# Yusheng-Xu/VGS-SVGS-Segmentation

Measured on AMD Instinct MI355X. Metric: segmented points/sec (end-to-end VGS), higher is better.
Workload: dtype f32

## Files before the change

vgs-svgs-segmentation_amd/csrc/capi.hip:

```cpp
#include <algorithm>
#include <cstdio>
#include <cstdlib>
#include <cstring>
#include <fstream>
#include <string>
#include <vector>

#include <dlfcn.h>

#include "vgs_context.hpp"

static thread_local std::string g_create_err;

static const char* const VGS_STAGE_NAMES[VGS_T_COUNT] = {"vgs:voxelize", "vgs:features", "vgs:adjacency", "vgs:localcut", "vgs:merge", "vgs:labels",
                                                         "vgs:total", "vgs:localcut_kernel", "vgs:supervoxels", "vgs:localcut_bulk", "", ""};
struct RoctxApi {
  int (*push)(const char*) = nullptr;
  int (*pop)() = nullptr;
  RoctxApi() {
    for (const char* name : {"librocprofiler-sdk-roctx.so.1", "librocprofiler-sdk-roctx.so", "libroctx64.so.4", "libroctx64.so"}) {
      void* h = dlopen(name, RTLD_LAZY | RTLD_LOCAL);
      if (!h) continue;
      push = (int (*)(const char*))dlsym(h, "roctxRangePushA");
      pop = (int (*)())dlsym(h, "roctxRangePop");
// ... 92 lines not shown
  }
  auto num = [&](size_t k) -> double { return k < v.size() ? std::atof(v[k].c_str()) : 0.0; };
  auto inum = [&](size_t k) -> int { return k < v.size() ? std::atoi(v[k].c_str()) : 0; };
  if (v.size() < 51) return VGS_E_IO;
  const int method = inum(24);
  if (method == 3) {
    if (v.size() < 61) return VGS_E_IO;
    vgs_params_default_svgs(p);
    p->voxel_size = (float)num(28); p->seed_size = (float)num(30); p->graph_size = (float)num(32);
    p->sig_p = (float)num(34); p->sig_n = (float)num(36); p->sig_o = (float)num(38); p->sig_e = (float)num(40);
    p->sig_c = (float)num(42); p->sig_w = (float)num(44);
    p->color_impt = (float)num(46); p->spatial_impt = (float)num(48); p->normal_impt = (float)num(50);
    p->cut_thred = (float)num(52);
    p->points_min = (int)num(54); p->voxels_min = inum(58); p->adjacency_min = inum(60);
  } else {
    vgs_params_default_vgs(p);
    p->voxel_size = (float)num(28); p->graph_size = (float)num(30);
    p->sig_p = (float)num(32); p->sig_n = (float)num(34); p->sig_o = (float)num(36); p->sig_e = (float)num(38);
    p->sig_c = (float)num(40); p->sig_w = (float)num(42); p->cut_thred = (float)num(44);
    p->points_min = inum(46); p->adjacency_min = inum(48); p->voxels_min = inum(50);
    p->method = 2;
  }
  if (in_name && name_cap > 0) { std::strncpy(in_name, v[15].c_str(), name_cap - 1); in_name[name_cap - 1] = 0; }
  if (out_name && name_cap > 0) { std::strncpy(out_name, v[21].c_str(), name_cap - 1); out_name[name_cap - 1] = 0; }
  return VGS_OK;
}

vgs_status vgs_create(const vgs_params* p, vgs_ctx** out) {
  if (!p || !out) return VGS_E_ARG;
  *out = nullptr;
  if (!(p->voxel_size > 0.f) || !(p->graph_size > 0.f) || !(p->sig_w != 0.f) || (p->method != 2 && p->method != 3)) {
    g_create_err = "vgs_create: voxel_size, graph_size must be > 0, sig_w != 0, method 2 or 3";
    return VGS_E_ARG;
  }
  if (p->vccs_mode != 0 && p->vccs_mode != 1) { g_create_err = "vgs_create: vccs_mode must be 0 (synchronous variant) or 1 (PCL's order)"; return VGS_E_ARG; }
  int ndev = 0;
  hipError_t e = hipGetDeviceCount(&ndev);
  if (e != hipSuccess || ndev <= 0) {
    g_create_err = std::string("vgs_create: no HIP device (") + hipGetErrorString(e) + "); this engine has no CPU path";
    return VGS_E_HIP;
  }
  if (p->device < 0 || p->device >= ndev) { g_create_err = "vgs_create: bad device ordinal"; return VGS_E_ARG; }
  vgs_ctx* c = new (std::nothrow) vgs_ctx();
  if (!c) return VGS_E_NOMEM;
  c->P = *p;
  c->device = p->device;
  int prio_lo = 0, prio_hi = 0;
  if (hipSetDevice(c->device) != hipSuccess || hipStreamCreateWithFlags(&c->stream, hipStreamNonBlocking) != hipSuccess ||
      hipDeviceGetStreamPriorityRange(&prio_lo, &prio_hi) != hipSuccess ||
      hipStreamCreateWithPriority(&c->stream2, hipStreamNonBlocking, prio_hi) != hipSuccess ||
      hipStreamCreateWithPriority(&c->stream3, hipStreamNonBlocking, prio_hi) != hipSuccess ||
      hipStreamCreateWithPriority(&c->stream4, hipStreamNonBlocking, prio_hi) != hipSuccess) {
    g_create_err = "vgs_create: hipSetDevice/hipStreamCreate failed";
    vgs_destroy(c);
    return VGS_E_HIP;
  }
  if (hipHostMalloc(&c->pin, 4096, hipHostMallocDefault) != hipSuccess) c->pin = nullptr;
  bool ok = hipStreamCreateWithFlags(&c->s_h2d, hipStreamNonBlocking) == hipSuccess &&
            hipStreamCreateWithFlags(&c->s_d2h, hipStreamNonBlocking) == hipSuccess &&
            hipEventCreateWithFlags(&c->ev_h2d, hipEventDisableTiming) == hipSuccess &&
            hipEventCreateWithFlags(&c->ev_d2h, hipEventDisableTiming) == hipSuccess &&
            hipEventCreateWithFlags(&c->ev_rb, hipEventDisableTiming) == hipSuccess &&
            hipEventCreateWithFlags(&c->ev_ho, hipEventDisableTiming) == hipSuccess &&
            hipEventCreateWithFlags(&c->ev_ho2, hipEventDisableTiming) == hipSuccess;
  for (int i = 0; ok && i < 16; ++i) ok = hipEventCreate(&c->ev[i]) == hipSuccess;
  for (int i = 0; ok && i < VGS_T_COUNT; ++i) ok = hipEventCreate(&c->tev[i][0]) == hipSuccess && hipEventCreate(&c->tev[i][1]) == hipSuccess;
  if (!ok) { g_create_err = "vgs_create: hipStreamCreate/hipEventCreate failed"; vgs_destroy(c); return VGS_E_HIP; }
  vgs_read_env_knobs(c);
  *out = c;
  return VGS_OK;
}

void vgs_destroy(vgs_ctx* c) {
  if (!c) return;
  (void)hipSetDevice(c->device);
  if (c->stream) (void)hipStreamSynchronize(c->stream);
  if (c->stream2) (void)hipStreamSynchronize(c->stream2);
  if (c->stream3) (void)hipStreamSynchronize(c->stream3);
  if (c->stream4) (void)hipStreamSynchronize(c->stream4);
  if (c->s_h2d) (void)hipStreamSynchronize(c->s_h2d);
  if (c->s_d2h) (void)hipStreamSynchronize(c->s_d2h);
  c->xyz_buf[0].release(); c->xyz_buf[1].release(); c->pt_label_alt.release(); c->grow_state.release();
  c->code_a.release(); c->code_b.release(); c->perm_a.release(); c->perm_b.release(); c->sort_tmp.release();
  c->head_flag.release(); c->pt_vox.release(); c->vox_code.release(); c->vox_start.release();
  c->xs.release(); c->ys.release(); c->zs.release();
  c->node.release(); c->used_ids.release(); c->used_rank.release();
  c->hkey.release(); c->hval.release(); c->offsets.release(); c->adj_masks.release(); c->adj_gtab.release(); c->adj_nvals.release(); c->adj_nrank.release(); c->adj_key.release(); c->adj_off.release(); c->adj_cnt.release(); c->adj_mused.release();
  c->nl_cnt.release(); c->nl_tot.release(); c->nl_ent.release(); c->lc_ctab.release(); c->pl_state.release(); c->pl_ent.release(); c->pl_work.release();
  c->sd_key.release(); c->sd_ids.release(); c->sd_vp.release(); c->sd_seg.release(); c->sd_tmp.release(); c->sd_part.release();
  c->sd_npts.release(); c->sd_nnodes.release(); c->sd_bbox.release(); c->sd_eig8.release(); c->sd_cen.release(); c->sd_cov.release(); c->sd_eval.release(); c->sd_evec.release();
  c->sd_apos.release(); c->sd_mom.release();
  c->sg_lab.release(); c->sg_nrec.release(); c->sg_ridx.release(); c->sg_ework.release(); c->sg_meta.release(); c->sg_roff.release(); c->sg_rkey.release(); c->sg_rec.release(); c->sg_part.release(); c->sg_tmp.release();
  c->sg_ab.release(); c->sg_nodes.release(); c->sg_npairs.release(); c->sg_nfin.release(); c->sg_wsum.release(); c->sg_wmin.release(); c->sg_wmax.release();
  c->cl_off.release(); c->cl_idx.release(); c->conn.release(); c->evals.release(); c->lc_pending.release(); c->lc_defer.release(); c->lc_defer_flag.release(); c->csize.release(); c->attach.release(); c->cc_flags.release(); c->parent.release(); c->csz.release();
  c->vc_cen.release(); c->vc_nrm.release(); c->vc_dist.release(); c->vc_state.release(); c->vc_tile_start.release(); c->vc_cell.release(); c->vc_plive.release(); c->vc_tile_of.release(); c->vc_tchg.release(); c->vc_nbr_tiles.release(); c->vc_halo.release(); c->vc_tile_meta.release(); c->vc_pool.release(); c->vc_ring.release(); c->vc_dbg.release(); c->vc_label.release();
  c->vc_seedkey.release(); c->vc_sums.release(); c->vc_count.release(); c->vc_accu.release(); c->vc_alive.release();
  c->sv_label.release(); c->sv_key_a.release(); c->sv_key_b.release(); c->cell_code_a.release(); c->cell_code_b.release();
  c->cell_id_a.release(); c->cell_id_b.release(); c->cell_start.release();
  c->owned.release(); c->straddle.release(); c->mixsrc.release(); c->bnd_code.release(); c->bnd_root.release(); c->root_label.release();
  c->bnd_code2.release(); c->bnd_root2.release(); c->bnd_cnt.release(); c->broot.release();
  c->kept_rank.release(); c->vox_label.release(); c->pt_label.release(); c->counters.release(); c->work_ids.release();
  if (c->pin) (void)hipHostFree(c->pin);
  for (int i = 0; i < 16; ++i) if (c->ev[i]) (void)hipEventDestroy(c->ev[i]);
  for (int i = 0; i < VGS_T_COUNT; ++i) for (int k = 0; k < 2; ++k) if (c->tev[i][k]) (void)hipEventDestroy(c->tev[i][k]);
  if (c->stream) (void)hipStreamDestroy(c->stream);
  if (c->stream2) (void)hipStreamDestroy(c->stream2);
  if (c->stream3) (void)hipStreamDestroy(c->stream3);
  if (c->stream4) (void)hipStreamDestroy(c->stream4);
  if (c->s_h2d) (void)hipStreamDestroy(c->s_h2d);
  if (c->s_d2h) (void)hipStreamDestroy(c->s_d2h);
  if (c->ev_h2d) (void)hipEventDestroy(c->ev_h2d);
  if (c->ev_rb) (void)hipEventDestroy(c->ev_rb);
  if (c->ev_ho) (void)hipEventDestroy(c->ev_ho);
  if (c->ev_ho2) (void)hipEventDestroy(c->ev_ho2);
  if (c->ev_d2h) (void)hipEventDestroy(c->ev_d2h);
  delete c;
}

vgs_status vgs_set_params(vgs_ctx* c, const vgs_params* p) {
  if (!c || !p) return VGS_E_ARG;
  if (!(p->voxel_size > 0.f) || !(p->graph_size > 0.f) || !(p->sig_w != 0.f)) { c->err = "vgs_set_params: voxel_size, graph_size > 0, sig_w != 0"; return VGS_E_ARG; }
  if (p->method != c->P.method || p->device != c->P.device) { c->err = "vgs_set_params: method and device are fixed at vgs_create"; return VGS_E_ARG; }
  if (p->vccs_mode != 0 && p->vccs_mode != 1) { c->err = "vgs_set_params: vccs_mode must be 0 (synchronous variant) or 1 (PCL's order)"; return VGS_E_ARG; }
  int keep = ST_SEGMENTED;
  const vgs_params& o = c->P;
  if (p->cut_thred != o.cut_thred || p->sig_p != o.sig_p || p->sig_n != o.sig_n || p->sig_o != o.sig_o || p->sig_e != o.sig_e ||
      p->sig_c != o.sig_c || p->sig_w != o.sig_w || p->adjacency_min != o.adjacency_min || p->voxels_min != o.voxels_min ||
      p->q7_count_as_index != o.q7_count_as_index)
    keep = ST_ADJACENCY;
  if (p->graph_size != o.graph_size) keep = ST_FEATURES;
  if (p->points_min != o.points_min) keep = ST_VOXELS;
  if (p->voxel_size != o.voxel_size || p->seed_size != o.seed_size || p->color_impt != o.color_impt ||
      p->spatial_impt != o.spatial_impt || p->normal_impt != o.normal_impt || p->vccs_mode != o.vccs_mode)
    keep = ST_POINTS;
  if (c->stage > keep) c->stage = keep;
  if (keep < ST_SEGMENTED) { c->sd_valid = false; c->sg_valid = false; c->sg_halo_valid = false; c->sg_own_K = -1; }
  if (keep == ST_POINTS && c->P.method == 3 && !c->sv_labels_external) { c->sv_have_labels = false; c->sv_max_label = 0; c->sv_label_n = -1; }
  c->P = *p;
  return VGS_OK;
}

const char* vgs_last_error_string(const vgs_ctx* c) { return c ? c->err.c_str() : g_create_err.c_str(); }

static vgs_status set_points_common(vgs_ctx* c, int64_t n, int32_t stride_bytes) {
  if (n < 0 || (stride_bytes != 12 && stride_bytes != 16)) { c->err = "set_points: n >= 0 and stride_bytes 12 or 16 required"; return VGS_E_ARG; }
  if (n >= (int64_t)1 << 31) { c->err = "set_points: more than 2^31-1 points"; return VGS_E_UNSUPPORTED; }
  c->N = n;
  c->stride_f = stride_bytes / 4;
  c->stage = ST_POINTS;
  c->sd_valid = false;
  c->sg_valid = false; c->sg_halo_valid = false; c->sg_own_K = -1;
  c->grid_covers = false;
  c->counts[VGS_N_POINTS] = n;
  for (int i = 0; i < VGS_T_COUNT; ++i) { c->times[i] = 0; c->tev_pending[i] = false; }
  c->sv_have_labels = false; c->sv_labels_external = false; c->sv_max_label = 0; c->sv_label_n = -1;
  c->n_own = -1; c->own_first = 0;
  return VGS_OK;
}

vgs_status vgs_set_points(vgs_ctx* c, const float* xyz_host, int64_t n, int32_t stride_bytes) {
  if (!c || (!xyz_host && n > 0)) return VGS_E_ARG;
  VGS_HIP_TRY(c, hipSetDevice(c->device));
  vgs_status s = set_points_common(c, n, stride_bytes);
  if (s != VGS_OK) return s;
  DevBuf<float>& buf = c->xyz_buf[c->xyz_cur];
  VGS_HIP_TRY(c, buf.ensure((size_t)n * c->stride_f + 4));
  if (n > 0) VGS_HIP_TRY(c, hipMemcpyAsync(buf.p, xyz_host, (size_t)n * stride_bytes, hipMemcpyHostToDevice, c->stream));
// ... 514 lines not shown
```

vgs-svgs-segmentation_amd/csrc/vgs_context.hpp:

```cpp
#ifndef VGS_CONTEXT_HPP_
#define VGS_CONTEXT_HPP_

#include <hip/hip_runtime.h>
#include <stdint.h>
#include <string.h>

#include <string>
#include <vector>

#include "../../include/vgs.h"
#include "vgs_math.h"
#include "pairlist.hpp"

typedef VgsNode NodeRec;
static_assert(sizeof(NodeRec) == 64, "NodeRec must be 64 bytes");

#ifdef __HIPCC__
__device__ __forceinline__ int64_t vgs_xcd_item(unsigned int b, int64_t n) {
  const int64_t per = (n + 7) >> 3;
  return (int64_t)(b & 7u) * per + (int64_t)(b >> 3);
}
#endif
static inline unsigned int vgs_xcd_grid(int64_t n) { return (unsigned int)(((n + 7) >> 3) << 3); }

// ... 35 lines not shown
  double w_sum;
  uint32_t cnt_lt, n_finite;
  int32_t a, b;
  float w_min, w_max;
};
struct SgPart {
  double w_sum;
  int64_t n_pairs, n_finite;
  int32_t nodes_a, nodes_b;
  float w_min, w_max;
};

enum Stage { ST_NONE = 0, ST_POINTS = 1, ST_VOXELS = 2, ST_FEATURES = 3, ST_ADJACENCY = 4, ST_SEGMENTED = 5 };

struct VgsKnobs {
  int a1_max = 4;
  float shell0 = 8.0f;
  float cap_frac = 0.7f;
  int dbg_stop = 0;
  int max_rounds = 6;
  int dbg_max_m = 0;
  int dbg_xl_from = 0;
  int near_min_own = 7;
  int fv_blocks = 512;
  int only_class = -1;
  bool no_dense = false;
  bool no_overlap = false;
  bool no_near = false;
  bool no_adjmasks = false;
  int vote_period = 64;
  int cross_lds_kb = 0;
  bool no_sort32 = false;
  bool no_pg_xl = false;
  bool no_connbits = false;
  bool no_pairlists = false;
  bool no_vote = false;
  int vote_force = 0;
  int ho_grid = -1;
  int pg_min_frac = 8;
  int pg_wide = 1;
  int pg_wide_frac = 8;
  bool debug = false;
};

struct vgs_ctx {
  vgs_params P;
  VgsKnobs K;
  int device = 0;
  hipStream_t stream = nullptr;
  hipStream_t stream2 = nullptr;
  hipStream_t stream3 = nullptr;
  hipStream_t stream4 = nullptr;
  std::string err;
  int stage = ST_NONE;
  void* pin = nullptr;

  const float* xyz = nullptr;
  DevBuf<float> xyz_buf[2];
  int xyz_cur = 0;
  hipStream_t s_h2d = nullptr, s_d2h = nullptr;
  hipEvent_t ev_h2d = nullptr, ev_d2h = nullptr;
  hipEvent_t ev_rb = nullptr;
  bool gathered = false;
  bool bricks_ready = false;
  bool staged = false;
  int64_t staged_n = 0;
  int staged_stride = 12;
  bool pt_labels_pending = false;
  bool labels_event_valid = false;
  bool d2h_open = false;
  const int32_t* d2h_src = nullptr;
  int64_t N = 0;
  int stride_f = 3;

  OctreeBox box;
  bool grid_pinned = false;
  bool grid_covers = false;
  int n_epochs = 0;

  DevBuf<uint64_t> code_a, code_b;
  DevBuf<uint32_t> perm_a, perm_b;
  DevBuf<uint8_t> sort_tmp;
  DevBuf<uint64_t> grow_state;
  DevBuf<uint32_t> head_flag, pt_vox;
  DevBuf<uint64_t> vox_code;
  DevBuf<uint32_t> vox_start;
  DevBuf<float> xs, ys, zs;
  int64_t Nf = 0;
  int64_t V = 0;
  int code_bits = 0;

  DevBuf<NodeRec> node;
  DevBuf<uint32_t> used_ids, used_rank;
  int64_t U = 0;

  DevBuf<uint64_t> hkey;
  DevBuf<uint32_t> hval;
  uint32_t hbits = 0;
  DevBuf<int32_t> offsets;
  DevBuf<uint64_t> adj_masks;
  int adj_mask_nb = 0;
  bool adj_tab_valid = false;
  float adj_tab_graph = 0.f, adj_tab_voxel = 0.f;
  DevBuf<uint16_t> adj_gtab;
  DevBuf<int32_t> adj_nvals;
  DevBuf<uint8_t> adj_nrank;
  int adj_ngroups = 0, adj_gstride = 0;
  bool adj_have_gtab = false;
  int n_off = 0;
  int adj_R = 0;
  int adj_stride = 0;
  DevBuf<uint64_t> adj_key;
  DevBuf<uint16_t> adj_off;
  bool adj_have_off = false;
  DevBuf<uint32_t> conn_bits;
  int cb_words = 0, cb_R = 0;
  bool cb_enabled = false;
  DevBuf<uint32_t> adj_cnt, adj_mused;
  bool adj_pruned = false;
  float adj_r2 = 0.f;

  DevBuf<uint8_t> nl_cnt;
  DevBuf<uint32_t> nl_tot;
  DevBuf<float4> nl_ent;
  bool nl_enabled = false;
  int nl_reach_steps = 0;
  bool nl_direct = false;

  DevBuf<uint8_t> pl_state;
  DevBuf<float4> pl_ent;
  DevBuf<uint32_t> pl_work;
  bool pl_enabled = false;
  bool pl_enabled_at_launch = false;
  hipEvent_t ev_ho = nullptr, ev_ho2 = nullptr;
  float pl_w_ring = 0.0f;

  DevBuf<uint8_t> conn;
  DevBuf<uint32_t> evals;
  DevBuf<uint8_t> lc_pending;
  DevBuf<uint8_t> lc_defer_flag;
  DevBuf<uint32_t> lc_defer;
  struct { bool open = false; bool dense = true; bool gated = false;  bool many = false;  unsigned int grid_f = 0, grid_g = 0, nabc[5] = {0, 0, 0, 0, 0}; float tail_ms = 0.f; bool pg_xl_queued = false;  } lc_tail;
  int64_t lc_diag[16] = {0};
  DevBuf<float> lc_ctab;
  float lc_ctab_key[8] = {0}, lc_ctab_scale = 0.0f;
  bool lc_ctab_valid = false;
  DevBuf<uint32_t> csize;
  DevBuf<int32_t> attach;
  DevBuf<uint8_t> cc_flags;
  DevBuf<uint32_t> parent;
  DevBuf<uint32_t> csz, kept_rank;
  DevBuf<int32_t> vox_label;
  DevBuf<int32_t> pt_label;
  DevBuf<int32_t> pt_label_alt;
  DevBuf<int64_t> cl_off;
  DevBuf<int32_t> cl_idx;
  bool cl_valid = false;
  DevBuf<uint32_t> sd_key, sd_ids, sd_vp, sd_seg;
  DevBuf<uint8_t> sd_tmp;
  DevBuf<double> sd_part;
  DevBuf<int64_t> sd_npts;
  DevBuf<int32_t> sd_nnodes;
  DevBuf<float> sd_bbox, sd_eig8;
  DevBuf<double> sd_cen, sd_cov, sd_eval, sd_evec;
  bool sd_valid = false;
  DevBuf<uint32_t> sd_apos;
  DevBuf<double> sd_mom;
// ... 139 lines not shown
```

vgs-svgs-segmentation_amd/csrc/voxelize.hip:

```cpp
#include <cstddef>
#include <cstdlib>
#include <cstring>
#include <string.h>

#include <rocprim/rocprim.hpp>

#include <algorithm>
#include <cmath>
#include <limits>

#include "vgs_context.hpp"

bool OctreeBox::contains(const float* p) const {
  if (!defined) return false;
  for (int a = 0; a < 3; ++a)
    if ((double)p[a] < min[a] || (double)p[a] >= max[a]) return false;
  return true;
}

void OctreeBox::adopt(const float* p) {
  const double eps = (double)std::numeric_limits<float>::epsilon();
  while (true) {
    if (!defined) {
      for (int a = 0; a < 3; ++a) { min[a] = (double)p[a] - res / 2; max[a] = (double)p[a] + res / 2; }
// ... 116 lines not shown
    double side = (double)(1u << g->depth) * res;
    for (int a = 0; a < 3; ++a)
      if (!hi[a]) { g->min[a] -= side; g->shift[a] += (1ull << g->depth); }
    g->depth++;
    side = (double)(1u << g->depth) * res - eps;
    for (int a = 0; a < 3; ++a) g->max[a] = g->min[a] + side;
    if (g->depth > 30) break;
  }
  if (g->record) {
    if (g->n_epochs >= VGS_MAX_EPOCHS) { g->overflow = 1; g->done = 1; return; }
    Epoch& e = g->epochs[g->n_epochs++];
    e.first = (int64_t)idx;
    for (int a = 0; a < 3; ++a) { e.min[a] = g->min[a]; e.shift[a] = g->shift[a]; }
  }
  g->start = (long long)idx + 1;
}
__global__ void k_adopt(const float* __restrict__ xyz, int stride_f, GrowState* __restrict__ g, int pinned) {
  if (g->done) return;
  const unsigned long long idx = g->found;
  g->found = ~0ull;
  if (idx == ~0ull) { g->done = 1; return; }
  if (pinned) { g->done = 2; return; }
  grow_adopt(xyz, stride_f, g, idx);
}

__global__ __launch_bounds__(1024) void k_grow_prefix(const float* __restrict__ xyz, int stride_f, int64_t n_prefix, GrowState* __restrict__ gs, int pinned) {
  __shared__ GrowState S;
  __shared__ unsigned long long s_best[16];
  const int tid = threadIdx.x;
  static_assert(sizeof(GrowState) % 8 == 0, "copied as 64-bit words");
  for (int k = tid; k < (int)(sizeof(GrowState) / 8); k += 1024) ((unsigned long long*)&S)[k] = ((const unsigned long long*)gs)[k];
  __syncthreads();
  if (S.done) return;
  while (true) {
    BoxD box;
    for (int a = 0; a < 3; ++a) { box.min[a] = S.min[a]; box.max[a] = S.max[a]; }
    box.defined = S.defined;
    const int64_t start = S.start;
    unsigned long long best = ~0ull;
    for (int64_t i = start + tid; i < n_prefix; i += 1024) {
      const float* p = xyz + i * stride_f;
      if (fv_outside(p[0], p[1], p[2], box)) { best = (unsigned long long)i; break; }
    }
    for (int o = 32; o > 0; o >>= 1) { const unsigned long long other = __shfl_down(best, o, 64); best = other < best ? other : best; }
    __syncthreads();
    if ((tid & 63) == 0) s_best[tid >> 6] = best;
    __syncthreads();
    if (tid == 0) {
      unsigned long long b = ~0ull;
      for (int w = 0; w < 16; ++w) b = s_best[w] < b ? s_best[w] : b;
      if (b == ~0ull) { if (S.start < n_prefix) S.start = n_prefix; S.found = ~0ull; s_best[0] = 0ull; }
      else if (pinned) { S.done = 2; s_best[0] = 0ull; }
      else { grow_adopt(xyz, stride_f, &S, b); s_best[0] = (S.done || S.overflow) ? 0ull : 1ull; }
    }
    __syncthreads();
    if (s_best[0] == 0ull) break;
    __syncthreads();
  }
  for (int k = tid; k < (int)(sizeof(GrowState) / 8); k += 1024) ((unsigned long long*)gs)[k] = ((const unsigned long long*)&S)[k];
}

template <typename KeyT>
__global__ void k_make_codes(const float* __restrict__ xyz, int stride_f, int64_t n, const GrowState* __restrict__ gs,
                             double res, int code_bits, KeyT* __restrict__ code, uint32_t* __restrict__ perm, int pack_shift) {
  int64_t i = (int64_t)blockIdx.x * blockDim.x + threadIdx.x;
  if (i >= n) return;
  const float* p = xyz + i * stride_f;
  float x = p[0], y = p[1], z = p[2];
  uint64_t c = 0;
  if (finite3(x, y, z)) {
    int e = gs->n_epochs - 1;
    while (e > 0 && i < gs->epochs[e].first) --e;
    const Epoch& ep = gs->epochs[e];
    uint32_t kx = vm_axis_key(x, ep.min[0], res) + (uint32_t)(gs->shift[0] - ep.shift[0]);
    uint32_t ky = vm_axis_key(y, ep.min[1], res) + (uint32_t)(gs->shift[1] - ep.shift[1]);
    uint32_t kz = vm_axis_key(z, ep.min[2], res) + (uint32_t)(gs->shift[2] - ep.shift[2]);
    c = (1ull << code_bits) | vm_morton(kx, ky, kz);
  }
  if (pack_shift > 0) { code[i] = (KeyT)((c << pack_shift) | (uint64_t)i); return; }
  code[i] = (KeyT)c;
  perm[i] = (uint32_t)i;
}

template <typename KeyT>
__global__ void k_heads(const KeyT* __restrict__ code, int64_t n, uint32_t* __restrict__ head, int pack_shift, uint32_t* __restrict__ perm_out) {
  int64_t j = (int64_t)blockIdx.x * blockDim.x + threadIdx.x;
  if (j < n) {
    const uint64_t raw = (uint64_t)code[j];
    const uint64_t c = raw >> pack_shift;
    head[j] = (c != 0 && (j == 0 || ((uint64_t)code[j - 1] >> pack_shift) != c)) ? 1u : 0u;
    if (pack_shift > 0) perm_out[j] = (uint32_t)(raw & ((1ull << pack_shift) - 1ull));
  }
}

template <typename KeyT>
__global__ void k_count_valid(const KeyT* __restrict__ code, int64_t n, unsigned long long* __restrict__ n_valid, int pack_shift) {
  int64_t lo = 0, hi = n;
  while (lo < hi) { int64_t mid = (lo + hi) >> 1; if (((uint64_t)code[mid] >> pack_shift) != 0) lo = mid + 1; else hi = mid; }
  *n_valid = (unsigned long long)lo;
}
__global__ void k_copy_last(const uint32_t* __restrict__ scan, int64_t n, unsigned long long* __restrict__ out) { *out = (unsigned long long)scan[n - 1]; }

template <typename KeyT>
__global__ void k_voxel_table(const KeyT* __restrict__ code, const uint32_t* __restrict__ head,
                              const uint32_t* __restrict__ scan, int64_t n, uint64_t mask, uint32_t* __restrict__ pt_vox,
                              uint64_t* __restrict__ vox_code, uint32_t* __restrict__ vox_start, int pack_shift) {
  int64_t j = (int64_t)blockIdx.x * blockDim.x + threadIdx.x;
  if (j >= n) return;
  uint64_t c = (uint64_t)code[j] >> pack_shift;
  if (c == 0) { pt_vox[j] = 0xffffffffu; return; }
  uint32_t v = scan[j] - 1u;
  pt_vox[j] = v;
  if (head[j]) { vox_code[v] = c & mask; vox_start[v] = (uint32_t)j; }
}

__global__ void k_gather_points(const float* __restrict__ xyz, int stride_f, const uint32_t* __restrict__ perm, int64_t nf,
                                float* __restrict__ xs, float* __restrict__ ys, float* __restrict__ zs) {
  int64_t j = (int64_t)blockIdx.x * blockDim.x + threadIdx.x;
  if (j >= nf) return;
  const float* p = xyz + (int64_t)perm[j] * stride_f;
  xs[j] = p[0]; ys[j] = p[1]; zs[j] = p[2];
}

__global__ void k_set_u32(uint32_t* p, uint32_t v) { *p = v; }

vgs_status vgs_grow_box_from(vgs_ctx* c, OctreeBox& box, bool record_epochs) {
  static_assert(sizeof(GrowState) % 8 == 0, "GrowState is copied as 64-bit words");
  VGS_HIP_TRY(c, c->counters.ensure(64));
  VGS_HIP_TRY(c, c->grow_state.ensure(sizeof(GrowState) / 8));
  GrowState* d_g = (GrowState*)c->grow_state.p;
  static thread_local GrowState h;
  std::memset(&h, 0, sizeof(h));
  for (int a = 0; a < 3; ++a) { h.min[a] = box.min[a]; h.max[a] = box.max[a]; h.shift[a] = box.shift[a]; }
  h.res = box.res; h.depth = box.depth; h.defined = box.defined ? 1 : 0;
  h.found = ~0ull; h.start = 0; h.record = record_epochs ? 1 : 0;
  const size_t hb_bytes = offsetof(GrowState, epochs) + sizeof(Epoch);
  const bool covering = c->grid_pinned && c->grid_covers && record_epochs && box.defined;
  if (covering) h.done = 1;
  if (record_epochs && box.defined) {
    Epoch& e = h.epochs[h.n_epochs++];
    e.first = 0;
    for (int a = 0; a < 3; ++a) { e.min[a] = box.min[a]; e.shift[a] = box.shift[a]; }
  }
  {
    const size_t hb = hb_bytes;
    static_assert(offsetof(GrowState, epochs) + sizeof(Epoch) <= 1024, "the growth header fits its slot of the pinned scratch");
    const void* src = &h;
    if (c->pin) { memcpy((char*)c->pin + 1024, &h, hb); src = (char*)c->pin + 1024; }
    VGS_HIP_TRY(c, hipMemcpyAsync(d_g, src, hb, hipMemcpyHostToDevice, c->stream));
  }
  if (covering) {
    c->n_epochs = h.n_epochs;
    return VGS_OK;
  }
  const int pinned = (c->grid_pinned && record_epochs) ? 1 : 0;
  const int blocks = (int)std::max<int64_t>(8, std::min<int64_t>((c->N / 4 + 255) / 256 + 1, (int64_t)c->K.fv_blocks));
  hipLaunchKernelGGL(k_grow_prefix, dim3(1), dim3(1024), 0, c->stream, c->xyz, c->stride_f, std::min<int64_t>(c->N, 8192), d_g, pinned);
  for (int batch = 0; batch < 64; ++batch) {
    for (int k = 0; k < (batch == 0 ? 2 : 8); ++k) {
      hipLaunchKernelGGL(k_first_violation, dim3(blocks), dim3(256), 0, c->stream, c->xyz, c->stride_f, c->N, d_g);
      hipLaunchKernelGGL(k_adopt, dim3(1), dim3(1), 0, c->stream, c->xyz, c->stride_f, d_g, pinned);
    }
    VGS_READBACK(c, &h, d_g, offsetof(GrowState, epochs));
    if (h.done) break;
  }
  if (h.done == 2) { c->err = "a point lies outside the pinned grid"; return VGS_E_ARG; }
  if (h.overflow || !h.done) { c->err = "octree grew more than VGS_MAX_EPOCHS times"; return VGS_E_UNSUPPORTED; }
  for (int a = 0; a < 3; ++a) { box.min[a] = h.min[a]; box.max[a] = h.max[a]; box.shift[a] = h.shift[a]; }
  box.depth = h.depth; box.defined = h.defined != 0;
  if (record_epochs) c->n_epochs = h.n_epochs;
  return VGS_OK;
}

static vgs_status grow_box(vgs_ctx* c) {
  if (!c->grid_pinned) {
    c->box = OctreeBox();
    c->box.res = (double)c->P.voxel_size;
  }
  return vgs_grow_box_from(c, c->box, true);
}

template <typename KeyT>
static vgs_status voxelize_sorted_table(vgs_ctx* c) {
  const int64_t N = c->N;
  const int TB = 256;
  const unsigned nb = (unsigned)((N + TB - 1) / TB);
  KeyT* code_a = (KeyT*)c->code_a.p;
  KeyT* code_b = (KeyT*)c->code_b.p;
  const unsigned key_bits = (unsigned)(c->code_bits + 1);
  int idx_bits = 1;
  while (idx_bits < 32 && ((int64_t)1 << idx_bits) < N) ++idx_bits;
  const int pack_shift = (sizeof(KeyT) == 8 && (int)key_bits + idx_bits <= 64) ? idx_bits : 0;
  hipLaunchKernelGGL((k_make_codes<KeyT>), dim3(nb), dim3(TB), 0, c->stream, c->xyz, c->stride_f, N, (const GrowState*)c->grow_state.p, c->box.res,
                     c->code_bits, code_a, c->perm_a.p, pack_shift);

  using nine_bits = rocprim::radix_sort_config<rocprim::default_config, rocprim::default_config,
                                               rocprim::radix_sort_onesweep_config<rocprim::kernel_config<1024, 6>, rocprim::kernel_config<1024, 6>, 9,
                                                                                   rocprim::block_radix_rank_algorithm::match>>;
  const bool use9 = (key_bits + 8) / 9 < (key_bits + 7) / 8;
  auto sort_pairs = [&](void* tmp, size_t& bytes) -> hipError_t {
    if (pack_shift > 0)
      return use9 ? rocprim::radix_sort_keys_desc<nine_bits>(tmp, bytes, code_a, code_b, (size_t)N, (unsigned)pack_shift, (unsigned)pack_shift + key_bits, c->stream)
                  : rocprim::radix_sort_keys_desc(tmp, bytes, code_a, code_b, (size_t)N, (unsigned)pack_shift, (unsigned)pack_shift + key_bits, c->stream);
    return use9 ? rocprim::radix_sort_pairs_desc<nine_bits>(tmp, bytes, code_a, code_b, c->perm_a.p, c->perm_b.p, (size_t)N, 0, key_bits, c->stream)
                : rocprim::radix_sort_pairs_desc(tmp, bytes, code_a, code_b, c->perm_a.p, c->perm_b.p, (size_t)N, 0, key_bits, c->stream);
  };
  size_t tmp_bytes = 0;
  VGS_HIP_TRY(c, sort_pairs(nullptr, tmp_bytes));
  size_t scan_bytes = 0;
  VGS_HIP_TRY(c, rocprim::inclusive_scan(nullptr, scan_bytes, c->head_flag.p, c->perm_a.p, (size_t)N, rocprim::plus<uint32_t>(), c->stream));
  VGS_HIP_TRY(c, c->sort_tmp.ensure(std::max(tmp_bytes, scan_bytes)));
  VGS_HIP_TRY(c, sort_pairs(c->sort_tmp.p, tmp_bytes));
  unsigned long long* d_cnt = (unsigned long long*)c->counters.p;
  VGS_HIP_TRY(c, hipMemsetAsync(d_cnt, 0, 2 * sizeof(unsigned long long), c->stream));
  hipLaunchKernelGGL((k_heads<KeyT>), dim3(nb), dim3(TB), 0, c->stream, code_b, N, c->head_flag.p, pack_shift, c->perm_b.p);
  hipLaunchKernelGGL((k_count_valid<KeyT>), dim3(1), dim3(1), 0, c->stream, code_b, N, d_cnt, pack_shift);
  uint32_t* scan = c->perm_a.p;
  VGS_HIP_TRY(c, rocprim::inclusive_scan(c->sort_tmp.p, scan_bytes, c->head_flag.p, scan, (size_t)N, rocprim::plus<uint32_t>(), c->stream));
  hipLaunchKernelGGL(k_copy_last, dim3(1), dim3(1), 0, c->stream, scan, N, d_cnt + 1);
  unsigned long long h2[2] = {0, 0};
  if (vgs_can_split_readback(c)) {
    { vgs_status sb = vgs_readback_begin(c, d_cnt, sizeof(h2)); if (sb != VGS_OK) return sb; }
    VGS_HIP_TRY(c, c->xs.ensure(N + 1)); VGS_HIP_TRY(c, c->ys.ensure(N + 1)); VGS_HIP_TRY(c, c->zs.ensure(N + 1));
    hipLaunchKernelGGL(k_gather_points, dim3(nb), dim3(TB), 0, c->stream, c->xyz, c->stride_f, c->perm_b.p, N, c->xs.p, c->ys.p, c->zs.p);
    c->gathered = true;
    { vgs_status se = vgs_readback_end(c, h2, sizeof(h2)); if (se != VGS_OK) return se; }
  } else {
    VGS_READBACK(c, h2, d_cnt, sizeof(h2));
  }
  const unsigned long long nf = h2[0];
  const uint32_t v_total = (uint32_t)h2[1];
  c->Nf = (int64_t)nf;
  c->V = (int64_t)v_total;
  VGS_HIP_TRY(c, c->vox_code.ensure(c->V + 1)); VGS_HIP_TRY(c, c->vox_start.ensure(c->V + 1));
  const uint64_t mask = (c->code_bits >= 64) ? ~0ull : ((1ull << c->code_bits) - 1ull);
  hipLaunchKernelGGL((k_voxel_table<KeyT>), dim3(nb), dim3(TB), 0, c->stream, code_b, c->head_flag.p, scan, N, mask, c->pt_vox.p,
                     c->vox_code.p, c->vox_start.p, pack_shift);
  hipLaunchKernelGGL(k_set_u32, dim3(1), dim3(1), 0, c->stream, c->vox_start.p + c->V, (uint32_t)c->Nf);
  return VGS_OK;
}

vgs_status vgs_stage_voxelize(vgs_ctx* c) {
  const int64_t N = c->N;
  c->V = 0; c->Nf = 0; c->U = 0;
  vgs_status st = grow_box(c);
  if (st != VGS_OK) return st;
  if (c->n_epochs == 0) {
    c->counts[VGS_N_FINITE] = 0; c->counts[VGS_N_VOXELS] = 0; c->counts[VGS_N_DEPTH] = 0;
    return VGS_OK;
  }
  if (c->box.depth > 21) { c->err = "octree depth > 21 (64-bit voxel codes exhausted)"; return VGS_E_UNSUPPORTED; }
  c->code_bits = 3 * c->box.depth;

  VGS_HIP_TRY(c, c->code_a.ensure(N)); VGS_HIP_TRY(c, c->code_b.ensure(N));
  VGS_HIP_TRY(c, c->perm_a.ensure(N)); VGS_HIP_TRY(c, c->perm_b.ensure(N));
  VGS_HIP_TRY(c, c->head_flag.ensure(N)); VGS_HIP_TRY(c, c->pt_vox.ensure(N));
  const int TB = 256;
  c->gathered = false;
  st = (c->code_bits + 1 <= 32) ? voxelize_sorted_table<uint32_t>(c) : voxelize_sorted_table<uint64_t>(c);
  if (st != VGS_OK) return st;
  if (!c->gathered) { VGS_HIP_TRY(c, c->xs.ensure(c->Nf + 1)); VGS_HIP_TRY(c, c->ys.ensure(c->Nf + 1)); VGS_HIP_TRY(c, c->zs.ensure(c->Nf + 1)); }
  if (c->Nf > 0 && !c->gathered) {
    const unsigned nbf = (unsigned)((c->Nf + TB - 1) / TB);
    hipLaunchKernelGGL(k_gather_points, dim3(nbf), dim3(TB), 0, c->stream, c->xyz, c->stride_f, c->perm_b.p, c->Nf, c->xs.p, c->ys.p,
                       c->zs.p);
  }
  VGS_HIP_TRY(c, hipGetLastError());
  c->counts[VGS_N_FINITE] = c->Nf;
  c->counts[VGS_N_VOXELS] = c->V;
  c->counts[VGS_N_DEPTH] = c->box.depth;
  return VGS_OK;
}
```

Baseline: 1.595 billion.

## Replace head-flag scan pipeline with tiled run-count and fused voxel-run kernels

Replaces the per-point head-flag kernel, rocprim inclusive scan, binary-search valid count and copy-last kernels with a three-step tiled scheme. The first pass counts run heads and valid points per 2048-key tile with vectorized loads. A single-block kernel then prefix-sums the tile counts. The final pass recomputes the heads and writes voxel ids, codes and starts using a wave-level scan. This removes the head_flag and scan arrays and several launches, cutting memory traffic. In exchange the keys are read twice, and the one-block tile-offset kernel runs serially over many tiles for large N.

```diff
diff --git a/vgs-svgs-segmentation_amd/csrc/capi.hip b/vgs-svgs-segmentation_amd/csrc/capi.hip
--- a/vgs-svgs-segmentation_amd/csrc/capi.hip
+++ b/vgs-svgs-segmentation_amd/csrc/capi.hip
@@ -198,7 +198,7 @@
   if (c->s_d2h) (void)hipStreamSynchronize(c->s_d2h);
   c->xyz_buf[0].release(); c->xyz_buf[1].release(); c->pt_label_alt.release(); c->grow_state.release();
   c->code_a.release(); c->code_b.release(); c->perm_a.release(); c->perm_b.release(); c->sort_tmp.release();
-  c->head_flag.release(); c->pt_vox.release(); c->vox_code.release(); c->vox_start.release();
+  c->head_flag.release(); c->pt_vox.release(); c->vox_tile.release(); c->vox_code.release(); c->vox_start.release();
   c->xs.release(); c->ys.release(); c->zs.release();
   c->node.release(); c->used_ids.release(); c->used_rank.release();
   c->hkey.release(); c->hval.release(); c->offsets.release(); c->adj_masks.release(); c->adj_gtab.release(); c->adj_nvals.release(); c->adj_nrank.release(); c->adj_key.release(); c->adj_off.release(); c->adj_cnt.release(); c->adj_mused.release();
diff --git a/vgs-svgs-segmentation_amd/csrc/vgs_context.hpp b/vgs-svgs-segmentation_amd/csrc/vgs_context.hpp
--- a/vgs-svgs-segmentation_amd/csrc/vgs_context.hpp
+++ b/vgs-svgs-segmentation_amd/csrc/vgs_context.hpp
@@ -141,7 +141,9 @@
   DevBuf<uint32_t> perm_a, perm_b;
   DevBuf<uint8_t> sort_tmp;
   DevBuf<uint64_t> grow_state;
-  DevBuf<uint32_t> head_flag, pt_vox;
+  DevBuf<uint32_t> pt_vox;
+  DevBuf<uint32_t> vox_tile;
+  DevBuf<uint32_t> head_flag;
   DevBuf<uint64_t> vox_code;
   DevBuf<uint32_t> vox_start;
   DevBuf<float> xs, ys, zs;
diff --git a/vgs-svgs-segmentation_amd/csrc/voxelize.hip b/vgs-svgs-segmentation_amd/csrc/voxelize.hip
--- a/vgs-svgs-segmentation_amd/csrc/voxelize.hip
+++ b/vgs-svgs-segmentation_amd/csrc/voxelize.hip
@@ -222,36 +222,132 @@
   perm[i] = (uint32_t)i;
 }
 
+#define VR_TB 512
+#define VR_KPT 4
+#define VR_TILE (VR_TB * VR_KPT)
+
 template <typename KeyT>
-__global__ void k_heads(const KeyT* __restrict__ code, int64_t n, uint32_t* __restrict__ head, int pack_shift, uint32_t* __restrict__ perm_out) {
-  int64_t j = (int64_t)blockIdx.x * blockDim.x + threadIdx.x;
-  if (j < n) {
-    const uint64_t raw = (uint64_t)code[j];
-    const uint64_t c = raw >> pack_shift;
-    head[j] = (c != 0 && (j == 0 || ((uint64_t)code[j - 1] >> pack_shift) != c)) ? 1u : 0u;
-    if (pack_shift > 0) perm_out[j] = (uint32_t)(raw & ((1ull << pack_shift) - 1ull));
-  }
+__device__ __forceinline__ void vr_load(const KeyT* __restrict__ code, int64_t n, int64_t j0, KeyT (&k)[VR_KPT], KeyT& prev) {
+  struct alignas(sizeof(KeyT) * VR_KPT) Vec { KeyT v[VR_KPT]; };
+  if (j0 + VR_KPT <= n) {
+    const Vec q = *(const Vec*)(code + j0);
+#pragma unroll
+    for (int i = 0; i < VR_KPT; ++i) k[i] = q.v[i];
+  } else {
+#pragma unroll
+    for (int i = 0; i < VR_KPT; ++i) k[i] = (j0 + i < n) ? code[j0 + i] : (KeyT)0;
+  }
+  prev = (KeyT)__shfl_up(k[VR_KPT - 1], 1, 64);
+  if ((threadIdx.x & 63) == 0) prev = (j0 > 0 && j0 < n) ? code[j0 - 1] : (KeyT)0;
+}
+__device__ __forceinline__ uint32_t vr_flags(const uint64_t (&c)[VR_KPT], uint64_t cprev, bool first, uint32_t& valid) {
+  uint32_t m = 0;
+  valid = 0;
+#pragma unroll
+  for (int i = 0; i < VR_KPT; ++i) {
+    const uint64_t before = i == 0 ? cprev : c[i - 1];
+    if (c[i] != 0) { ++valid; if ((i == 0 && first) || before != c[i]) m |= 1u << i; }
+  }
+  return m;
 }
 
 template <typename KeyT>
-__global__ void k_count_valid(const KeyT* __restrict__ code, int64_t n, unsigned long long* __restrict__ n_valid, int pack_shift) {
-  int64_t lo = 0, hi = n;
-  while (lo < hi) { int64_t mid = (lo + hi) >> 1; if (((uint64_t)code[mid] >> pack_shift) != 0) lo = mid + 1; else hi = mid; }
-  *n_valid = (unsigned long long)lo;
-}
-__global__ void k_copy_last(const uint32_t* __restrict__ scan, int64_t n, unsigned long long* __restrict__ out) { *out = (unsigned long long)scan[n - 1]; }
+__global__ __launch_bounds__(VR_TB) void k_run_counts(const KeyT* __restrict__ code, int64_t n, int pack_shift, uint32_t* __restrict__ perm_out,
+                                                      uint32_t* __restrict__ tile_heads, uint32_t* __restrict__ tile_valid) {
+  __shared__ uint32_t s_h[VR_TB / 64], s_v[VR_TB / 64];
+  const int64_t j0 = (int64_t)blockIdx.x * VR_TILE + (int64_t)threadIdx.x * VR_KPT;
+  KeyT k[VR_KPT], kp;
+  vr_load(code, n, j0, k, kp);
+  uint64_t c[VR_KPT];
+#pragma unroll
+  for (int i = 0; i < VR_KPT; ++i) c[i] = (uint64_t)k[i] >> pack_shift;
+  uint32_t valid;
+  uint32_t heads = (uint32_t)__popc(vr_flags(c, (uint64_t)kp >> pack_shift, j0 == 0, valid));
+  if (pack_shift > 0) {
+    const uint64_t low = (1ull << pack_shift) - 1ull;
+    if (j0 + VR_KPT <= n) {
+      *(uint4*)(perm_out + j0) = make_uint4((uint32_t)((uint64_t)k[0] & low), (uint32_t)((uint64_t)k[1] & low), (uint32_t)((uint64_t)k[2] & low),
+                                            (uint32_t)((uint64_t)k[3] & low));
+    } else {
+#pragma unroll
+      for (int i = 0; i < VR_KPT; ++i) if (j0 + i < n) perm_out[j0 + i] = (uint32_t)((uint64_t)k[i] & low);
+    }
+  }
+  for (int o = 32; o > 0; o >>= 1) { heads += __shfl_down(heads, o, 64); valid += __shfl_down(valid, o, 64); }
+  if ((threadIdx.x & 63) == 0) { s_h[threadIdx.x >> 6] = heads; s_v[threadIdx.x >> 6] = valid; }
+  __syncthreads();
+  if (threadIdx.x == 0) {
+    uint32_t h = 0, v = 0;
+    for (int w = 0; w < VR_TB / 64; ++w) { h += s_h[w]; v += s_v[w]; }
+    tile_heads[blockIdx.x] = h;
+    tile_valid[blockIdx.x] = v;
+  }
+}
+static_assert(VR_KPT == 4, "k_run_counts and k_voxel_runs store four 32-bit words per thread at once");
+
+__global__ __launch_bounds__(1024) void k_tile_offsets(uint32_t* __restrict__ tile_heads, const uint32_t* __restrict__ tile_valid, int64_t n_tiles,
+                                                       unsigned long long* __restrict__ cnt) {
+  __shared__ unsigned long long s_h[1024], s_v[16];
+  const int tid = threadIdx.x;
+  const int64_t per = (n_tiles + 1023) / 1024;
+  const int64_t lo = (int64_t)tid * per < n_tiles ? (int64_t)tid * per : n_tiles, hi = lo + per < n_tiles ? lo + per : n_tiles;
+  unsigned long long h = 0, v = 0;
+  for (int64_t t = lo; t < hi; ++t) { h += tile_heads[t]; v += tile_valid[t]; }
+  s_h[tid] = h;
+  for (int o = 32; o > 0; o >>= 1) v += __shfl_down(v, o, 64);
+  if ((tid & 63) == 0) s_v[tid >> 6] = v;
+  __syncthreads();
+  for (int o = 1; o < 1024; o <<= 1) {
+    const unsigned long long add = tid >= o ? s_h[tid - o] : 0ull;
+    __syncthreads();
+    s_h[tid] += add;
+    __syncthreads();
+  }
+  uint32_t run = (uint32_t)(s_h[tid] - h);
+  for (int64_t t = lo; t < hi; ++t) { const uint32_t x = tile_heads[t]; tile_heads[t] = run; run += x; }
+  if (tid == 0) {
+    unsigned long long vt = 0;
+    for (int w = 0; w < 16; ++w) vt += s_v[w];
+    cnt[0] = vt;
+    cnt[1] = s_h[1023];
+  }
+}
 
 template <typename KeyT>
-__global__ void k_voxel_table(const KeyT* __restrict__ code, const uint32_t* __restrict__ head,
-                              const uint32_t* __restrict__ scan, int64_t n, uint64_t mask, uint32_t* __restrict__ pt_vox,
-                              uint64_t* __restrict__ vox_code, uint32_t* __restrict__ vox_start, int pack_shift) {
-  int64_t j = (int64_t)blockIdx.x * blockDim.x + threadIdx.x;
-  if (j >= n) return;
-  uint64_t c = (uint64_t)code[j] >> pack_shift;
-  if (c == 0) { pt_vox[j] = 0xffffffffu; return; }
-  uint32_t v = scan[j] - 1u;
-  pt_vox[j] = v;
-  if (head[j]) { vox_code[v] = c & mask; vox_start[v] = (uint32_t)j; }
+__global__ __launch_bounds__(VR_TB) void k_voxel_runs(const KeyT* __restrict__ code, int64_t n, int pack_shift, const uint32_t* __restrict__ tile_off,
+                                                      uint64_t mask, uint32_t* __restrict__ pt_vox, uint64_t* __restrict__ vox_code,
+                                                      uint32_t* __restrict__ vox_start, uint32_t n_vox, uint32_t n_finite) {
+  __shared__ uint32_t s_w[VR_TB / 64];
+  const int64_t j0 = (int64_t)blockIdx.x * VR_TILE + (int64_t)threadIdx.x * VR_KPT;
+  KeyT k[VR_KPT], kp;
+  vr_load(code, n, j0, k, kp);
+  uint64_t c[VR_KPT];
+#pragma unroll
+  for (int i = 0; i < VR_KPT; ++i) c[i] = (uint64_t)k[i] >> pack_shift;
+  uint32_t valid;
+  const uint32_t m = vr_flags(c, (uint64_t)kp >> pack_shift, j0 == 0, valid);
+  const uint32_t mine = (uint32_t)__popc(m);
+  uint32_t incl = mine;
+  const int lane = threadIdx.x & 63, wave = threadIdx.x >> 6;
+  for (int o = 1; o < 64; o <<= 1) { const uint32_t up = __shfl_up(incl, o, 64); if (lane >= o) incl += up; }
+  if (lane == 63) s_w[wave] = incl;
+  __syncthreads();
+  uint32_t run = tile_off[blockIdx.x] + incl - mine;
+  for (int w = 0; w < wave; ++w) run += s_w[w];
+  if (blockIdx.x == 0 && threadIdx.x == 0) vox_start[n_vox] = n_finite;
+  if (j0 >= n) return;
+  uint32_t out[VR_KPT];
+#pragma unroll
+  for (int i = 0; i < VR_KPT; ++i) {
+    if ((m >> i) & 1u) { vox_code[run] = c[i] & mask; vox_start[run] = (uint32_t)(j0 + i); ++run; }
+    out[i] = c[i] != 0 ? run - 1u : 0xffffffffu;
+  }
+  if (j0 + VR_KPT <= n) {
+    *(uint4*)(pt_vox + j0) = make_uint4(out[0], out[1], out[2], out[3]);
+  } else {
+#pragma unroll
+    for (int i = 0; i < VR_KPT; ++i) if (j0 + i < n) pt_vox[j0 + i] = out[i];
+  }
 }
 
 __global__ void k_gather_points(const float* __restrict__ xyz, int stride_f, const uint32_t* __restrict__ perm, int64_t nf,
@@ -261,8 +357,6 @@
   const float* p = xyz + (int64_t)perm[j] * stride_f;
   xs[j] = p[0]; ys[j] = p[1]; zs[j] = p[2];
 }
-
-__global__ void k_set_u32(uint32_t* p, uint32_t v) { *p = v; }
 
 vgs_status vgs_grow_box_from(vgs_ctx* c, OctreeBox& box, bool record_epochs) {
   static_assert(sizeof(GrowState) % 8 == 0, "GrowState is copied as 64-bit words");
@@ -347,17 +441,15 @@
   };
   size_t tmp_bytes = 0;
   VGS_HIP_TRY(c, sort_pairs(nullptr, tmp_bytes));
-  size_t scan_bytes = 0;
-  VGS_HIP_TRY(c, rocprim::inclusive_scan(nullptr, scan_bytes, c->head_flag.p, c->perm_a.p, (size_t)N, rocprim::plus<uint32_t>(), c->stream));
-  VGS_HIP_TRY(c, c->sort_tmp.ensure(std::max(tmp_bytes, scan_bytes)));
+  VGS_HIP_TRY(c, c->sort_tmp.ensure(tmp_bytes));
   VGS_HIP_TRY(c, sort_pairs(c->sort_tmp.p, tmp_bytes));
+  const int64_t n_tiles = (N + VR_TILE - 1) / VR_TILE;
+  VGS_HIP_TRY(c, c->vox_tile.ensure((size_t)(2 * n_tiles)));
+  uint32_t* tile_heads = c->vox_tile.p;
+  uint32_t* tile_valid = c->vox_tile.p + n_tiles;
   unsigned long long* d_cnt = (unsigned long long*)c->counters.p;
-  VGS_HIP_TRY(c, hipMemsetAsync(d_cnt, 0, 2 * sizeof(unsigned long long), c->stream));
-  hipLaunchKernelGGL((k_heads<KeyT>), dim3(nb), dim3(TB), 0, c->stream, code_b, N, c->head_flag.p, pack_shift, c->perm_b.p);
-  hipLaunchKernelGGL((k_count_valid<KeyT>), dim3(1), dim3(1), 0, c->stream, code_b, N, d_cnt, pack_shift);
-  uint32_t* scan = c->perm_a.p;
-  VGS_HIP_TRY(c, rocprim::inclusive_scan(c->sort_tmp.p, scan_bytes, c->head_flag.p, scan, (size_t)N, rocprim::plus<uint32_t>(), c->stream));
-  hipLaunchKernelGGL(k_copy_last, dim3(1), dim3(1), 0, c->stream, scan, N, d_cnt + 1);
+  hipLaunchKernelGGL((k_run_counts<KeyT>), dim3((unsigned)n_tiles), dim3(VR_TB), 0, c->stream, code_b, N, pack_shift, c->perm_b.p, tile_heads, tile_valid);
+  hipLaunchKernelGGL(k_tile_offsets, dim3(1), dim3(1024), 0, c->stream, tile_heads, tile_valid, n_tiles, d_cnt);
   unsigned long long h2[2] = {0, 0};
   if (vgs_can_split_readback(c)) {
     { vgs_status sb = vgs_readback_begin(c, d_cnt, sizeof(h2)); if (sb != VGS_OK) return sb; }
@@ -374,9 +466,8 @@
   c->V = (int64_t)v_total;
   VGS_HIP_TRY(c, c->vox_code.ensure(c->V + 1)); VGS_HIP_TRY(c, c->vox_start.ensure(c->V + 1));
   const uint64_t mask = (c->code_bits >= 64) ? ~0ull : ((1ull << c->code_bits) - 1ull);
-  hipLaunchKernelGGL((k_voxel_table<KeyT>), dim3(nb), dim3(TB), 0, c->stream, code_b, c->head_flag.p, scan, N, mask, c->pt_vox.p,
-                     c->vox_code.p, c->vox_start.p, pack_shift);
-  hipLaunchKernelGGL(k_set_u32, dim3(1), dim3(1), 0, c->stream, c->vox_start.p + c->V, (uint32_t)c->Nf);
+  hipLaunchKernelGGL((k_voxel_runs<KeyT>), dim3((unsigned)n_tiles), dim3(VR_TB), 0, c->stream, code_b, N, pack_shift, tile_heads, mask, c->pt_vox.p,
+                     c->vox_code.p, c->vox_start.p, v_total, (uint32_t)c->Nf);
   return VGS_OK;
 }
 
@@ -394,7 +485,7 @@
 
   VGS_HIP_TRY(c, c->code_a.ensure(N)); VGS_HIP_TRY(c, c->code_b.ensure(N));
   VGS_HIP_TRY(c, c->perm_a.ensure(N)); VGS_HIP_TRY(c, c->perm_b.ensure(N));
-  VGS_HIP_TRY(c, c->head_flag.ensure(N)); VGS_HIP_TRY(c, c->pt_vox.ensure(N));
+  VGS_HIP_TRY(c, c->pt_vox.ensure(N));
   const int TB = 256;
   c->gathered = false;
   st = (c->code_bits + 1 <= 32) ? voxelize_sorted_table<uint32_t>(c) : voxelize_sorted_table<uint64_t>(c);
```

Measured after the change: 1.624 billion (median of 6 runs). 1.8% higher.
